# HandSomeWay/myGauHuman

Hardware: AMD Instinct MI355X
Metric: frames/sec fwd+bwd @1024^2, 200k Gaussians (higher is better)
Workload: dtype f32

## Files before the change

include/gsr.h:

```cpp
#ifndef GSR_H_INCLUDED
#define GSR_H_INCLUDED

#include <stddef.h>
#include <stdint.h>

#ifdef __cplusplus
extern "C" {
#endif

#define GSR_OK 0
#define GSR_EINVAL (-1)
#define GSR_EHIP (-2)
#define GSR_ENOMEM (-3)

typedef void *gsr_stream_t;
typedef char *(*gsr_alloc_fn)(void *user, size_t bytes);

int gsr_version(void);
int gsr_has_experiments(void);
const char *gsr_target_arch(void);
const char *gsr_last_error(void);

#define GSR_BINNING_GLOBAL_RADIX 0
#define GSR_BINNING_TILE_BUCKET 1
// ... 117 lines not shown

#define GSR_Q_DEPTHS 0
#define GSR_Q_MEANS2D 1
#define GSR_Q_CONIC_OPACITY 2
#define GSR_Q_RGB 3
#define GSR_Q_COV3D 4
#define GSR_Q_TILES_TOUCHED 5
#define GSR_Q_POINT_OFFSETS 6
#define GSR_Q_CLAMPED 7
#define GSR_Q_POINT_LIST 8
#define GSR_Q_KEYS_SORTED 9
#define GSR_Q_RANGES 10
#define GSR_Q_FINAL_T 11
#define GSR_Q_N_CONTRIB 12
#define GSR_Q_ORDER 13
int gsr_query_state(int what, int P, int R, int width, int height, const char *geom_buffer,
                    const char *binning_buffer, const char *image_buffer, void *dst, gsr_stream_t stream);

size_t gsr_dist2_workspace_bytes(int P);
int gsr_dist2(int P, const float *points, float *mean_dists, char *workspace, size_t workspace_bytes,
              gsr_stream_t stream);

size_t gsr_sort_workspace_bytes(size_t n);
int gsr_sort_pairs_u64(size_t n, const uint64_t *keys_in, uint64_t *keys_out, const uint32_t *vals_in,
                       uint32_t *vals_out, int end_bit, char *workspace, size_t workspace_bytes,
                       gsr_stream_t stream);
int gsr_sort_pairs_u32(size_t n, const uint32_t *keys_in, uint32_t *keys_out, const uint32_t *vals_in,
                       uint32_t *vals_out, int end_bit, char *workspace, size_t workspace_bytes,
                       gsr_stream_t stream);

// ... 291 lines not shown
```

mygauhuman_amd/_lib.py:

```python
import ctypes as C
import os

import torch

_HERE = os.path.dirname(os.path.abspath(__file__))
LIB_PATH = os.path.join(_HERE, "libgsr.so")

ALLOC_FN = C.CFUNCTYPE(C.c_void_p, C.c_void_p, C.c_size_t)


class Phase1LossStruct(C.Structure):
    _fields_ = [("gt_image", C.c_void_p), ("gt_normal", C.c_void_p), ("alpha_target", C.c_void_p), ("bound", C.c_void_p),
                ("w_image", C.c_float), ("w_alpha", C.c_float), ("w_normal", C.c_float), ("w_axis", C.c_float),
                ("normal_triple", C.c_int), ("axis_triple", C.c_int),
                ("color", C.c_void_p), ("alpha", C.c_void_p), ("extra_images", C.c_void_p), ("stats", C.c_void_p),
                ("upstream", C.c_void_p)]

PBR_MAX_LEVELS = 16


class PbrTexture(C.Structure):
    _fields_ = [("cube", C.c_int), ("channels", C.c_int), ("levels", C.c_int),
                ("width", C.c_int * PBR_MAX_LEVELS), ("height", C.c_int * PBR_MAX_LEVELS),
                ("data", C.c_void_p * PBR_MAX_LEVELS), ("grad", C.c_void_p * PBR_MAX_LEVELS)]
# ... 47 lines not shown
    "gsr_body_pose_backward", "gsr_lbs_offset_mlp_packed_floats_nb", "gsr_lbs_offset_mlp_pack_nb", "gsr_lbs_offset_mlp_forward_nb",
    "gsr_debug_lbs_offset_mlp_forward_bf16x3_nb", "gsr_lbs_offset_mlp_backward_workspace_floats_nb", "gsr_lbs_offset_mlp_backward_nb",
    "gsr_pbr_texture_forward", "gsr_pbr_texture_backward", "gsr_pbr_cube_mip_forward", "gsr_pbr_cube_mip_backward",
    "gsr_pbr_diffuse_forward", "gsr_pbr_diffuse_backward", "gsr_pbr_specular_forward", "gsr_pbr_specular_backward",
    "gsr_pbr_shade_forward", "gsr_pbr_shade_backward",
    "gsr_bake_grid_workspace_bytes", "gsr_bake_grid", "gsr_bake_plan_bytes", "gsr_bake_plan", "gsr_bake_visibility_workspace_bytes",
    "gsr_bake_visibility", "gsr_bake_expand", "gsr_bake_env_reduce",
    "gsr_pbr_loss_workspace_floats", "gsr_pbr_loss_forward", "gsr_pbr_loss_backward",
    "gsr_pose_refiner_forward", "gsr_pose_refiner_backward",
    "gsr_bounding_rect_workspace_ints", "gsr_bounding_rect", "gsr_ssim_crop_workspace_floats", "gsr_ssim_crop_forward",
    "gsr_ssim_crop_backward",
]

GSR_OK = 0
Q = dict(DEPTHS=0, MEANS2D=1, CONIC_OPACITY=2, RGB=3, COV3D=4, TILES_TOUCHED=5, POINT_OFFSETS=6, CLAMPED=7,
         POINT_LIST=8, KEYS_SORTED=9, RANGES=10, FINAL_T=11, N_CONTRIB=12, ORDER=13)
BINNING_GLOBAL_RADIX, BINNING_TILE_BUCKET = 0, 1
SH_F32, SH_F16 = 0, 1
N_EXTRA = 18
DEFAULT_BINNING = BINNING_TILE_BUCKET
DEFAULT_TILE_CULL = 1
DEFAULT_BWD_REDUCE = 3
DEFAULT_TILE_ORDER = 1
DEFAULT_BLEND_LAYOUT = 0
DEFAULT_BLEND_SEGMENTS = 8


class GsrError(RuntimeError):
    pass


# ... 250 lines not shown
```

mygauhuman_amd/csrc/blend_bwd.hip:

```cpp
#include "gsr_common.h"

namespace gsr {

__device__ __forceinline__ uint32_t xcd_remap_b(uint32_t bid, uint32_t n) {
  const uint32_t q = n / 8, r = n % 8, xcd = bid % 8, k = bid / 8;
  const uint32_t start = xcd < r ? xcd * (q + 1) : r * (q + 1) + (xcd - r) * q;
  return start + k;
}

template <int CTRL>
__device__ __forceinline__ float dpp_f(float v) {
  return __builtin_bit_cast(float, __builtin_amdgcn_update_dpp(0, __builtin_bit_cast(int, v), CTRL, 0xF, 0xF, false));
}
__device__ __forceinline__ float row16_sum(float v) {
  v += dpp_f<0xB1>(v);
  v += dpp_f<0x4E>(v);
  v += dpp_f<0x124>(v);
  v += dpp_f<0x128>(v);
  return v;
}
__device__ __forceinline__ float half8_sum(float v) {
  v += dpp_f<0xB1>(v);
  v += dpp_f<0x4E>(v);
  v += dpp_f<0x141>(v);
// ... 575 lines not shown
    dps[ch][1] = t4.y;
    dps[ch][2] = t4.z;
    dps[ch][3] = t4.w;
  }
  __builtin_amdgcn_wave_barrier();
  const float4 *rd_r = reinterpret_cast<const float4 *>(&s_rw[row * WAVE + kcol * 4u]);
  const float4 *rd_w = reinterpret_cast<const float4 *>(&s_rw[(4u + row) * WAVE + kcol * 4u]);
  constexpr uint32_t H2_QA = 68, H2_QB = 0, H2_QC = 132, H2_KA = 224, H2_KB = 292;
  constexpr uint64_t H2_P = ((uint64_t)(H2_QB / 4)) | ((uint64_t)((H2_QA + 8) / 4) << 7) | ((uint64_t)(H2_QC / 4) << 14) |
                            ((uint64_t)((H2_QB + 8) / 4) << 21) | ((uint64_t)((H2_QC + 8) / 4) << 28) | ((uint64_t)(H2_QA / 4) << 35) |
                            ((uint64_t)(H2_KA / 4) << 42) | ((uint64_t)((H2_KA + 8) / 4) << 49) | ((uint64_t)(H2_KB / 4) << 56);
  static_assert((H2_KB + WAVE) * 4 <= RW_BYTES, "hop 2 fits the reduction buffer");
  const uint32_t k9 = kcol < 9u ? kcol : 0u;
  const float4 *src8 = reinterpret_cast<const float4 *>(&s_rw[row * 16u + 4u * (uint32_t)((H2_P >> (7u * k9)) & 127u)]);

  uint32_t id_next = 0;
  if (skip + (int)lane < walk_end) id_next = a.point_list[range.y - 1 - (skip + (int)lane)];
  for (int base = skip; base < walk_end; base += WAVE) {
    const int idx = base + (int)lane;
    bool keep = false;
    float4 r0 = make_float4(0, 0, 0, 0), r1 = r0, r2 = r0;
    float l255 = 0.f;
    const uint32_t id = id_next;
    if (idx < walk_end) {
      const float4 *src = reinterpret_cast<const float4 *>(a.recs + id);
      r0 = src[0];
      r1 = src[1];
      r2 = src[2];
    }
    if (idx + WAVE < walk_end) id_next = a.point_list[range.y - 1 - (idx + WAVE)];
    if (idx < walk_end) {
      keep = (r0.x + r2.z >= rx0) && (r0.x - r2.z <= rx1) && (r0.y + r2.w >= ry0) && (r0.y - r2.w <= ry1);
      if (keep) {
        l255 = __builtin_amdgcn_logf(255.0f * r1.y);
        keep = ellipse_hits_rect_fast(r0.x, r0.y, r0.z, r0.w, r1.x, l255, rx0, rx1, ry0, ry1);
      }
    }
    const uint64_t kmask = __ballot(keep);
    const int cnt = __builtin_popcountll(kmask);
    if (keep) {
      const int slot = __builtin_popcountll(kmask & lt);
      constexpr float L2E = 1.4426950408889634f;
      s0[slot] = make_float4(r0.x, r0.y, (-0.5f * L2E) * r0.z, -L2E * r0.w);
      s1[slot] = make_float4((-0.5f * L2E) * r1.x, l255, __uint_as_float((uint32_t)(n - 1 - idx)), r1.y);
      s2[slot] = make_float4(r1.w, r2.x, r2.y, r1.z);
      s_id[slot] = id * (uint32_t)(GROW * sizeof(float));
    }
    __builtin_amdgcn_fence(__ATOMIC_RELEASE, "wavefront");
    __builtin_amdgcn_wave_barrier();
    __builtin_amdgcn_fence(__ATOMIC_ACQUIRE, "wavefront");

    uint32_t vg = 0u, vi = row * 4u;
    asm volatile("" : "+v"(vg), "+v"(vi));
    for (int g = 0; g < cnt; g += 4, vg += 64u, vi += 16u) {
      float ar[4], aw[4];
      uint32_t anyhit = 0;
#pragma unroll
      for (int u = 0; u < 4; u++) {
        bool done = false;
        if (g + u < cnt) {
          const float4 g0 = lds_at<float4>(s0, vg + 16u * u);
// ... 768 lines not shown
```

mygauhuman_amd/csrc/blend_fwd.hip:

```cpp
#include "gsr_common.h"
#include "tile_sort.h"

#ifndef FWD_FULL_ROWS
#define FWD_FULL_ROWS false
#endif
#ifndef FWD_FEATURE_WPG
#define FWD_FEATURE_WPG 2
#endif

namespace gsr {

__device__ __forceinline__ uint32_t xcd_remap(uint32_t bid, uint32_t n) {
  const uint32_t q = n / 8, r = n % 8, xcd = bid % 8, k = bid / 8;
  const uint32_t start = xcd < r ? xcd * (q + 1) : r * (q + 1) + (xcd - r) * q;
  return start + k;
}

template <int SLOTS, int CE>
constexpr int fwd_wpg() { return SLOTS == 1 ? (CE > 0 ? FWD_FEATURE_WPG : 4) : 1; }

__device__ __forceinline__ void workgroup_sort_tile(const uint64_t *b, int n, uint32_t tile, uint32_t base, uint32_t *point_list,
                                                    uint64_t *keys_sorted, uint32_t wv, uint32_t lane, uint64_t *s_runs,
                                                    uint32_t *s_ids) {
  const int nruns = (n + WAVE - 1) / WAVE, r0 = (int)wv, r1 = (int)wv + 4;
// ... 19 lines not shown
    if (r >= nruns) break;
    const uint64_t k = key[j];
    uint32_t rank = lane;
#pragma unroll
    for (int o = 0; o < MERGE_MAX_RUNS; o++)
      if (o != r && o < nruns) rank += rank_in_run(s_runs + o * WAVE, k);
    if (k != ~0ull) {
      point_list[base + rank] = (uint32_t)k;
      keys_sorted[base + rank] = ((uint64_t)tile << 32) | (k >> 32);
      s_ids[rank] = (uint32_t)k;
    }
  }
  __syncthreads();
}

template <int SLOTS, int CE>
__global__ __launch_bounds__((WAVE * fwd_wpg<SLOTS, CE>())) void blend_forward_kernel(const BlendFwdArgs a) {
  constexpr int WPG = fwd_wpg<SLOTS, CE>();
  constexpr uint32_t H = SLOTS == 1 ? 4 / WPG : 1;
  const uint32_t wv = threadIdx.x / WAVE;
  constexpr int WPT = 4 / SLOTS;
  constexpr int XS2 = CE > 0 ? (CE + 3) / 4 * 2 : 1;
  __shared__ __attribute__((aligned(16))) float2 s_x_all[CE > 0 ? WPG * WAVE * XS2 : 1];
  __shared__ float4 s0_all[WPG * WAVE];
  __shared__ float4 s1_all[WPG * WAVE];
  __shared__ float4 s2_all[WPG * WAVE];
  float2 *s_x = s_x_all + (CE > 0 ? wv * WAVE * XS2 : 0);
  float4 *s0 = s0_all + wv * WAVE, *s1 = s1_all + wv * WAVE, *s2 = s2_all + wv * WAVE;

  const unsigned long long trace_t0 = a.trace ? __builtin_amdgcn_s_memrealtime() : 0ull;
  uint32_t tile, part, nseg = 1;
  if constexpr (SLOTS == 1) {
// ... 46 lines not shown
    const int q = q0 + s;
    const int px = tx * TILE + (q & 1) * 8 + (int)(lane & 7);
    const int py = ty * TILE + (q >> 1) * 8 + (int)(lane >> 3);
    pxf[s] = (float)px;
    pyf[s] = (float)py;
    inside[s] = px < a.W && py < a.H;
    dbias[s] = inside[s] ? -0.02f : 1e30f;
    pixid[s] = py * a.W + px;
    T[s] = 1.0f;
    C0[s] = C1[s] = C2[s] = Dp[s] = Wt[s] = 0.f;
#pragma unroll
    for (int c = 0; c < (CE > 0 ? CE : 1); c++) X[s][c] = 0.f;
    last[s] = 0;
  }
  const uint64_t lt = lane == 0 ? 0ull : (~0ull >> (64 - lane));

  uint32_t id_a = 0, id_b = 0;
  float4 p0 = make_float4(0, 0, 0, 0), p1 = p0, p2 = p0;
  uint32_t id_cur = 0;
  if ((int)lane < n) {
    id_cur = list_at((int)lane);
    const float4 *src = reinterpret_cast<const float4 *>(a.recs + id_cur);
    p0 = src[0];
    p1 = src[1];
    p2 = src[2];
  }
  if ((int)lane + WAVE < n) id_a = list_at((int)lane + WAVE);
  const int seg_len = nseg > 1u ? segment_len(n, (int)nseg) : 0;
  uint32_t next_rec = 0;
  auto checkpoint = [&](uint32_t k) {
// ... 65 lines not shown
    };
    auto fetch_rest = [&](Row &r) {
      r.g2 = s2[r.kk];
      if (CE > 0) {
        const float4 *xr = reinterpret_cast<const float4 *>(&s_x[r.kk * XS2]);
#pragma unroll
        for (int c = 0; c < XS2 / 2; c++) r.x[c] = xr[c];
      }
    };
    auto fetch = [&](Row &r, int k) {
      r.kk = min(k, WAVE - 1);
      r.g0 = s0[r.kk];
      r.g1 = s1[r.kk];
      if constexpr (FULL) fetch_rest(r);
    };
    auto blend_one = [&](Row &r) {
#pragma unroll
      for (int s = 0; s < SLOTS; s++) {
        const float dx = r.g0.x - pxf[s], dy = r.g0.y - pyf[s];
        const float p2 = dx * (r.g0.z * dx + r.g0.w * dy) + (r.g1.x * dy) * dy;
        const bool pre = !(p2 > 0.0f) && ((p2 + r.g1.y) >= dbias[s]);
        if (__ballot(pre) != 0ull) {
          if constexpr (!FULL) fetch_rest(r);
          const float alpha = fminf(0.99f, r.g1.w * __builtin_amdgcn_exp2f(p2));
          const bool hit = pre && !(alpha < 1.0f / 255.0f);
          const float test_T = T[s] * (1.0f - alpha);
          const bool stop = hit && test_T < 0.0001f;
          const bool blend = hit && !stop;
          dbias[s] = stop ? 1e30f : dbias[s];
          const float w = blend ? alpha * T[s] : 0.0f;
          C0[s] += r.g2.x * w;
          C1[s] += r.g2.y * w;
          C2[s] += r.g2.z * w;
          Dp[s] += r.g2.w * w;
          Wt[s] += w;
          if (CE > 0) {
#pragma unroll
            for (int c = 0; c < CE; c++) {
              const float4 v = r.x[c / 4];
              X[s][c] += (c % 4 == 0 ? v.x : (c % 4 == 1 ? v.y : (c % 4 == 2 ? v.z : v.w))) * w;
            }
          }
          T[s] = blend ? test_T : T[s];
          last[s] = blend ? __float_as_uint(r.g1.z) : last[s];
        }
      }
    };
    Row A, B;
    fetch(A, 0);
    int k = 0;
    for (; k + 1 < cnt; k += 2) {
      fetch(B, k + 1);
      blend_one(A);
      fetch(A, k + 2);
      blend_one(B);
    }
    if (k < cnt) blend_one(A);
    __builtin_amdgcn_wave_barrier();
  }
  if (nseg > 1u)
    while (next_rec < nseg) checkpoint(next_rec++);
  if (a.trace && lane == 0) {
    unsigned long long *r = a.trace + ((size_t)blockIdx.x * WPG + wv) * 4u;
    r[0] = trace_t0;
    r[1] = __builtin_amdgcn_s_memrealtime();
    r[2] = (unsigned long long)n;
    r[3] = (unsigned long long)tile;
  }

  const size_t plane = (size_t)a.H * a.W;
  const float bg0 = a.bg[0], bg1 = a.bg[1], bg2 = a.bg[2];
#pragma unroll
// ... 27 lines not shown

constexpr int FX_PLANE16 = WAVE * 16;
constexpr int FX_BYTES = 4 * FX_PLANE16 + 2 * WAVE * 4;
constexpr int HALF = WAVE / 2;

__global__ __launch_bounds__(WAVE * 4) void blend_forward_features_kernel(const BlendFwdArgs a) {
  constexpr int CE = CE_MAX;
  const uint32_t wv = threadIdx.x / WAVE;
  __shared__ __attribute__((aligned(16))) char s_fx_all[4 * FX_BYTES];
  __shared__ float4 s0_all[4 * WAVE], s1_all[4 * WAVE], s2_all[4 * WAVE];
  __shared__ uint32_t s_lane_all[4 * WAVE];
  char *s_fx = s_fx_all + wv * FX_BYTES;
  float4 *s0w = s0_all + wv * WAVE, *s1w = s1_all + wv * WAVE, *s2w = s2_all + wv * WAVE;
  uint32_t *s_lanew = s_lane_all + wv * WAVE;
  const uint32_t fx_base = __builtin_amdgcn_readfirstlane((uint32_t)(uintptr_t)s_fx);

  const int omode = tile_order_mode(a.order);
  const uint32_t n_slots = tile_slots_of(a.order, a.grid_x, a.grid_y, omode);
  const uint32_t slot_id = omode ? blockIdx.x : (blockIdx.x < n_slots ? xcd_remap(blockIdx.x, n_slots) : n_slots);
  const uint32_t entry = tile_of_slot(a.order, omode, slot_id, n_slots), part = wv;
  if (entry == ORDER_NO_TILE || order_entry_seg(entry) != 0u) return;
  const uint32_t tile = order_entry_tile(entry);
  const int tx = tile % a.grid_x, ty = tile / a.grid_x;
  const uint32_t lane = threadIdx.x % WAVE;
  const uint2 range = a.ranges[tile];
  const int n = (int)(range.y - range.x);
  list_priority(a.order, n, a.list_prio);

  const int px = tx * TILE + (int)(part & 1) * 8 + (int)(lane & 7);
  const int py = ty * TILE + (int)(part >> 1) * 8 + (int)(lane >> 3);
// ... 142 lines not shown
  const uint32_t s = max(h.x, h.y);
  const fwd_u32x2 q = __builtin_amdgcn_permlane16_swap(s, s, false, false);
  return max(q.x, q.y);
}

template <int CE>
__global__ __launch_bounds__(WAVE * 4) void blend_forward_sp_kernel(const BlendFwdArgs a) {
  constexpr int XS = (CE + 3) / 4 * 4;
  __shared__ float4 s_x_all[CE > 0 ? 4 * WAVE * XS / 4 : 1];
  __shared__ float4 s0_all[4 * WAVE];
  __shared__ float4 s1_all[4 * WAVE];
  __shared__ float4 s2_all[4 * WAVE];
  const uint32_t wv = threadIdx.x / WAVE, lane = threadIdx.x % WAVE;
  float4 *s_x = s_x_all + (CE > 0 ? wv * WAVE * XS / 4 : 0);
  float4 *s0 = s0_all + wv * WAVE, *s1 = s1_all + wv * WAVE, *s2 = s2_all + wv * WAVE;

  const int omode = tile_order_mode(a.order);
  const uint32_t n_slots = tile_slots_of(a.order, a.grid_x, a.grid_y, omode);
  const uint32_t item = omode ? ordered_item4(blockIdx.x, n_slots) : (blockIdx.x < n_slots * 4u ? xcd_remap(blockIdx.x, n_slots * 4u) : n_slots * 4u);
  const uint32_t entry = tile_of_slot(a.order, omode, item / 4u, n_slots), quad = item % 4u;
  if (entry == ORDER_NO_TILE || order_entry_seg(entry) != 0u) return;
  const uint32_t tile = order_entry_tile(entry);
  const int tx = tile % a.grid_x, ty = tile / a.grid_x;
  const uint2 range = a.ranges[tile];
  const int n = (int)(range.y - range.x);
  list_priority(a.order, n, a.list_prio);

  s2[lane] = make_float4(0.f, 0.f, 0.f, 0.f);
  if (CE > 0) {
#pragma unroll
// ... 186 lines not shown
      return GSR_OK;
    }
#endif
    hipLaunchKernelGGL((blend_forward_kernel<1, CE_MAX>), dim3(slots * (4 / FWD_FEATURE_WPG)), dim3(WAVE * FWD_FEATURE_WPG), 0, stream, a);
    return GSR_OK;
  }
#ifdef GSR_BUILD_EXPERIMENTS
  if (opt.blend_layout == 1 && opt.blend_fwd_waves == 4) {
    hipLaunchKernelGGL((blend_forward_sp_kernel<0>), dim3(slots * 4), dim3(WAVE * 4), 0, stream, a);
    return GSR_OK;
  }
#endif
  switch (opt.blend_fwd_waves) {
    case 1: hipLaunchKernelGGL((blend_forward_kernel<4, 0>), dim3(tiles), dim3(WAVE), 0, stream, a); break;
    case 2: hipLaunchKernelGGL((blend_forward_kernel<2, 0>), dim3(tiles * 2), dim3(WAVE), 0, stream, a); break;
    default: hipLaunchKernelGGL((blend_forward_kernel<1, 0>), dim3(slots), dim3(WAVE * 4), 0, stream, a); break;
  }
  return GSR_OK;
}

}
```

mygauhuman_amd/csrc/gsr_api.hip:

```cpp
#include <stdarg.h>
#include <stdio.h>
#include <string.h>

#include <atomic>
#include <mutex>
#include <string>
#include <unordered_map>
#include <utility>
#include <vector>

#include "gsr_common.h"

namespace gsr {

static thread_local std::string g_error;

void set_error(const char *fmt, ...) {
  char buf[1024];
  va_list ap;
  va_start(ap, fmt);
  vsnprintf(buf, sizeof(buf), fmt, ap);
  va_end(ap);
  g_error = buf;
}
// ... 79 lines not shown
  } else if (!strcmp(key, "blend_bwd_waves")) {
    if (v != 1 && v != 2 && v != 4) return bad("1, 2 or 4");
    o.blend_bwd_waves = v;
  } else if (!strcmp(key, "bucket_cstride")) {
    if (v != 1 && v != 2 && v != 4 && v != 8 && v != 16) return bad("1, 2, 4, 8 or 16");
    o.bucket_cstride = v;
  } else if (!strcmp(key, "bucket_hist")) {
    if (v != 0 && v != 1) return bad("0 or 1");
    o.bucket_hist = v;
  } else if (!strcmp(key, "bucket_sort_merged")) {
    if (v != 0 && v != 1) return bad("0 or 1");
    o.bucket_sort_merged = v;
  } else if (!strcmp(key, "blend_sort")) {
    if (v != 0 && v != 1) return bad("0 or 1");
    o.blend_sort = v;
  } else if (!strcmp(key, "tile_order")) {
    if (v < 0 || v > 3) return bad("0 (natural order), 1 (longest lists first), 2 / 3 (2 x 2 / 4 x 2 tile blocks by summed length, a block per XCD)");
    o.tile_order = v;
  } else if (!strcmp(key, "tile_cull")) {
    if (v != 0 && v != 1) return bad("0 or 1");
    o.tile_cull = v;
  } else if (!strcmp(key, "blend_bwd_reduce")) {
    if (v < 0 || v > 4) return bad("0 (permlane / DPP folds), 3 (LDS folds: default); experiments: 1 (MFMA on folded rows), 2 (transposed MFMA contraction), 4 (LDS folds, the round-3 kernel)");
    if (experiment(v == 1 || v == 2 || v == 4)) return GSR_EINVAL;
    o.blend_bwd_reduce = v;
  } else if (!strcmp(key, "blend_layout")) {
    if (v != 0 && v != 1) return bad("0 (quadrant waves) or 1 (experiment: 4x4 blocks, four survivors per step)");
    if (experiment(v == 1)) return GSR_EINVAL;
    o.blend_layout = v;
  } else if (!strcmp(key, "blend_tail_cut")) {
// ... 336 lines not shown
  fa.W = in.width;
  fa.H = in.height;
  fa.grid_x = grid_x;
  fa.grid_y = grid_y;
  fa.bg = in.background;
  fa.out_color = in.out_color;
  fa.out_depth = in.out_depth;
  fa.out_alpha = in.out_alpha;
  fa.final_T = img.final_T;
  fa.n_contrib = img.n_contrib;
  fa.extra = in.extra;
  fa.CE = in.n_extra;
  fa.list_prio = opt.blend_prio;
  fa.ckpt_base = img.ckpt_base;
  fa.ckpt = img.ckpt;
  {
    ApiState &st = S();
    const size_t need = (size_t)tile_slots_max(grid_x, grid_y) * 4u * 4u;
    fa.trace = st.trace.load();
    if (fa.trace && st.trace_words.load() / 2 < need) {
      set_error("gsr_debug_wave_trace: the registered buffer holds %zu words, this image needs %zu (2 x 16 x visiting slots)",
                st.trace_words.load(), 2 * need);
      return GSR_EINVAL;
    }
  }
  fa.out_extra = in.out_extra;
  prof_begin(PROF_BLEND_FWD, stream);
  rc = launch_blend_forward(fa, opt, stream);
  prof_end(PROF_BLEND_FWD, stream);
  if (rc != GSR_OK) return rc;
// ... 166 lines not shown
  }
  if (p1 && (n_extra != CE_MAX || !p1->gt_image || !p1->gt_normal || !p1->alpha_target || !p1->bound || !p1->color || !p1->alpha ||
             !p1->extra_images || !p1->stats || p1->normal_triple < 0 || p1->normal_triple > 5 || p1->axis_triple < 0 ||
             p1->axis_triple > 5 || p1->axis_triple == p1->normal_triple)) {
    set_error("gsr_rasterize_backward_phase1_loss: the fused multi-feature pass (n_extra = %d), the forward's images, the targets, "
              "the bound mask, stats and two different triple indices in 0..5 are required", CE_MAX);
    return GSR_EINVAL;
  }
  if ((shs && !dL_dsh) || (scales && (!rotations || !dL_dscale || !dL_drot))) {
    set_error("gsr_rasterize_backward: missing gradient output for SH / scale / rotation inputs");
    return GSR_EINVAL;
  }
  const int grid_x = (width + TILE - 1) / TILE, grid_y = (height + TILE - 1) / TILE;
  const size_t tiles = (size_t)grid_x * grid_y, npix = (size_t)width * height;
  GeomState geom = geom_from_chunk(geom_buffer, (size_t)P);
  BinningState bin = binning_from_chunk(binning_buffer, (size_t)R);
  ImageState img = image_from_chunk(image_buffer, npix, tiles);
  if (!radii) radii = geom.internal_radii;

  if (n_extra != 0 && (n_extra != CE_MAX || !extra_features || !dL_dout_extra || !dL_dextra)) {
    set_error("gsr_rasterize_backward_ex: extra feature channels need n_extra == %d and all three arrays", CE_MAX);
    return GSR_EINVAL;
  }
  const int grow = n_extra ? GROWX : GROW;
  const Options opt = options_for(stream);
  float *det_rows = nullptr;
  const size_t det_bytes = (size_t)(R > 0 ? R : 1) * 4 * GROW * sizeof(float);
  if (opt.deterministic) {
    GSR_HIP(hipMalloc(reinterpret_cast<void **>(&det_rows), det_bytes));
    GSR_HIP(zero_async(det_rows, det_bytes, stream));
  } else if (!(flags & GSR_BWD_ROWS_ZEROED)) {
// ... 29 lines not shown
    if (ba.dL_dextra_tri[t]) ba.extra_mask |= 1u << t;
  }
  if (p1) {
    ba.p1 = *p1;
    ba.extra_mask |= (1u << p1->normal_triple) | (1u << p1->axis_triple);
    if (opt.deterministic || opt.blend_bwd_reduce != 3) {
      set_error("gsr_rasterize_backward_phase1_loss: built for the default reduction of the fused pass (blend_bwd_reduce = 3, not deterministic)");
      return GSR_EINVAL;
    }
  }
  ba.det_rows = det_rows;
  ba.debug_skip_atomics = opt.debug_no_atomics;
  ba.list_prio = opt.blend_prio;
  ba.ckpt_base = img.ckpt_base;
  ba.ckpt = img.ckpt;
  {
    ApiState &st = S();
    const size_t need = (size_t)tile_slots_max(ba.grid_x, ba.grid_y) * 4u * 4u;
    ba.trace = st.trace.load() ? st.trace.load() + st.trace_words.load() / 2 : nullptr;
    if (ba.trace && st.trace_words.load() / 2 < need) {
      set_error("gsr_debug_wave_trace: the registered buffer holds %zu words, this image needs %zu (2 x 16 x visiting slots)",
                st.trace_words.load(), 2 * need);
      return GSR_EINVAL;
    }
  }
  ba.radii = radii;
  ba.point_offsets = geom.point_offsets;
  ba.tiles_touched = geom.tiles_touched;
  prof_begin(PROF_BLEND_BWD, stream);
  int rc = launch_blend_backward(ba, opt, stream);
// ... 126 lines not shown
                           float *dL_dscale, float *dL_drot, int debug, gsr_stream_t stream) {
  return gsr_rasterize_backward_ex(P, D, M, R, background, width, height, means3D, shs, colors_precomp, alphas, scales,
                                   scale_modifier, rotations, cov3D_precomp, viewmatrix, projmatrix, campos, tan_fovx, tan_fovy,
                                   radii, geom_buffer, binning_buffer, image_buffer, dL_dpix, dL_ddepths, dL_dalphas, dL_dmean2D,
                                   dL_dconic, dL_dopacity, dL_dcolor, dL_dmean3D, dL_dcov3D, dL_dsh, dL_dscale, dL_drot, debug,
                                   nullptr, 0, nullptr, nullptr, GSR_SH_F32, stream);
}

int gsr_query_state(int what, int P, int R, int width, int height, const char *geom_buffer, const char *binning_buffer,
                    const char *image_buffer, void *dst, gsr_stream_t stream_) {
  hipStream_t stream = reinterpret_cast<hipStream_t>(stream_);
  const int grid_x = (width + TILE - 1) / TILE, grid_y = (height + TILE - 1) / TILE;
  const size_t tiles = (size_t)grid_x * grid_y, npix = (size_t)width * height;
  if (!dst) return GSR_EINVAL;
  GeomState geom = geom_from_chunk(const_cast<char *>(geom_buffer), (size_t)P);
  BinningState bin = binning_from_chunk(const_cast<char *>(binning_buffer), (size_t)R);
  ImageState img = image_from_chunk(const_cast<char *>(image_buffer), npix, tiles);
  const void *src = nullptr;
  size_t bytes = 0;
  switch (what) {
    case GSR_Q_DEPTHS:
    case GSR_Q_MEANS2D:
    case GSR_Q_CONIC_OPACITY:
    case GSR_Q_RGB:
    case GSR_Q_CLAMPED: {
      if (!geom_buffer) return GSR_EINVAL;
      int rc = launch_query_recs(what, P, geom, dst, stream);
      if (rc != GSR_OK) return rc;
      GSR_LAUNCH_CHECK(stream, 0);
      return GSR_OK;
    }
    case GSR_Q_COV3D: src = geom.cov3D; bytes = (size_t)P * 6 * 4; break;
    case GSR_Q_TILES_TOUCHED: src = geom.tiles_touched; bytes = (size_t)P * 4; break;
    case GSR_Q_POINT_OFFSETS: src = geom.point_offsets; bytes = (size_t)P * 4; break;
    case GSR_Q_POINT_LIST: src = bin.vals_s; bytes = (size_t)R * 4; break;
    case GSR_Q_KEYS_SORTED: src = bin.keys_s; bytes = (size_t)R * 8; break;
    case GSR_Q_RANGES: src = img.ranges; bytes = tiles * 8; break;
    case GSR_Q_FINAL_T: src = img.final_T; bytes = npix * 4; break;
    case GSR_Q_N_CONTRIB: src = img.n_contrib; bytes = npix * 4; break;
    case GSR_Q_ORDER: src = img.order; bytes = order_words(tiles) * 4; break;
    default: set_error("gsr_query_state: unknown selector %d", what); return GSR_EINVAL;
  }
  if (bytes) GSR_HIP(hipMemcpyAsync(dst, src, bytes, hipMemcpyDeviceToDevice, stream));
  return GSR_OK;
}

size_t gsr_sort_workspace_bytes(size_t n) {
  size_t m = n ? n : 1;
  return align_up(m * 8, 256) + align_up(m * 4, 256) + align_up(sort_hist_words(m) * 4, 256) + 1024;
}

static int sort_ws(size_t n, size_t key_bytes, char *ws, size_t ws_bytes, void **tk, uint32_t **tv, uint32_t **hist) {
  if (!ws || ws_bytes < gsr_sort_workspace_bytes(n)) {
    set_error("sort workspace too small (%zu < %zu)", ws_bytes, gsr_sort_workspace_bytes(n));
    return GSR_ENOMEM;
// ... 48 lines not shown
```

mygauhuman_amd/csrc/gsr_common.h:

```cpp
#pragma once
#include <hip/hip_runtime.h>
#include <stdint.h>
#include <stddef.h>

#include "../../include/gsr.h"

namespace gsr {

constexpr int TILE = 16;
constexpr int WAVE = 64;
constexpr int PRE_BLOCK = 256;

struct alignas(16) SplatRec {
  float x, y, conic_a, conic_b;
  float conic_c, opacity, depth, r;
  float g, b, hx, hy;
};
static_assert(sizeof(SplatRec) == 48, "SplatRec layout");

constexpr int GROW = 16;

constexpr int GROWX = 32;
constexpr int CE_MAX = 18;

// ... 6 lines not shown
  int *internal_radii;
  uint32_t *block_incl;
  uint32_t *block_sums;
  uint32_t *block_prefix;
  uint32_t *total;
  float *grad_rows;
};
struct BinningState {
  uint64_t *keys_a;
  uint32_t *vals_a;
  uint64_t *keys_s;
  uint32_t *vals_s;
  uint32_t *hist;
  uint32_t *tile_counts;
  uint32_t *tile_cursor;
};
struct ImageState {
  float *final_T;
  uint32_t *n_contrib;
  uint2 *ranges;
  uint32_t *order;
  uint32_t *ckpt_base;
  float *ckpt;
};

inline size_t align_up(size_t v, size_t a) { return (v + a - 1) / a * a; }
template <typename T>
inline void carve(uintptr_t &p, T *&out, size_t count) {
  p = align_up(p, 256);
  out = reinterpret_cast<T *>(p);
// ... 19 lines not shown
  carve(chunk, g.point_offsets, P);
  carve(chunk, g.internal_radii, P);
  carve(chunk, g.block_incl, P);
  carve(chunk, g.block_sums, nb);
  carve(chunk, g.block_prefix, nb);
  carve(chunk, g.total, 4);
  carve(chunk, g.grad_rows, P * GROWX);
  if (end) *end = chunk;
  return g;
}
inline size_t geom_bytes(size_t P) {
  size_t end = 0;
  geom_from_chunk(nullptr, P, &end);
  return end + 256;
}
inline BinningState binning_from_chunk(char *chunk_, size_t R, size_t tiles = 0, size_t *end = nullptr) {
  BinningState b;
  uintptr_t chunk = carve_begin(chunk_);
  size_t n = R ? R : 1;
  carve(chunk, b.keys_a, n);
  carve(chunk, b.vals_a, n);
  carve(chunk, b.keys_s, n);
  carve(chunk, b.vals_s, n);
  carve(chunk, b.hist, sort_hist_words(n));
  b.tile_counts = b.tile_cursor = nullptr;
  if (tiles) {
    carve(chunk, b.tile_counts, tiles * 16);
    carve(chunk, b.tile_cursor, tiles);
  }
  if (end) *end = chunk;
  return b;
}
inline size_t binning_bytes(size_t R, size_t tiles) {
  size_t end = 0;
  binning_from_chunk(nullptr, R, tiles ? tiles : 1, &end);
  return end + 256;
}
#if defined(__HIPCC__)
#define GSR_HD __host__ __device__
#else
#define GSR_HD
#endif
constexpr uint32_t ORDER_NO_TILE = 0xFFFFFFFFu;
// ... 56 lines not shown
    if (debug) GSR_HIP(hipStreamSynchronize(stream));                        \
  } while (0)

enum ProfStage { PROF_PREPROCESS_FWD = 0, PROF_SCAN = 1, PROF_BINNING = 2, PROF_BLEND_FWD = 3, PROF_BLEND_BWD = 4,
                 PROF_PREPROCESS_BWD = 5, PROF_NSTAGES = 6 };
void prof_begin(int stage, hipStream_t stream);
void prof_end(int stage, hipStream_t stream);

struct Options {
  int binning_mode = GSR_BINNING_TILE_BUCKET;
  int tile_cull = 1;
  int tile_order = 1;
  int bucket_hist = 1;
  int bucket_sort_merged = 1;
  int blend_sort = 1;
  int bucket_cstride = 4;
  int blend_fwd_dma = 0;
  int blend_fwd_waves = 4;
  int blend_bwd_waves = 4;
  int blend_bwd_reduce = 3;
  int deterministic = 0;
  int blend_layout = 0;
  int blend_tail_cut = 0;
  int blend_segments = 8;
  int blend_prio = 1;
  int bake_batch_cells = 0;
  int debug_no_atomics = 0;
};
Options options_for(hipStream_t stream);

// ... 27 lines not shown
  const uint2 *ranges;
  uint32_t *point_list;
  const SplatRec *recs;
  const uint64_t *unsorted;
  uint64_t *keys_sorted;
  int W, H, grid_x, grid_y;
  const float *bg;
  float *out_color, *out_depth, *out_alpha, *final_T;
  uint32_t *n_contrib;
  const float *extra;
  int CE;
  float *out_extra;
  int list_prio;
  const uint32_t *ckpt_base;
  float *ckpt;
  unsigned long long *trace;
};
int launch_blend_forward(const BlendFwdArgs &a, const Options &opt, hipStream_t stream);
bool forward_sorts_lists(const Options &opt, int n_extra);
__device__ __forceinline__ int tile_order_mode(const uint32_t *order) { return order ? (int)(order[0] & 0xFFu) : 0; }
__device__ __forceinline__ uint32_t tile_order_longest(const uint32_t *order) { return order ? order[0] >> 8 : 0u; }
__device__ __forceinline__ void list_priority(const uint32_t *order, int n, int enabled) {
  const uint32_t longest = tile_order_longest(order), n4 = 4u * (uint32_t)n;
  if (!enabled || longest == 0u) return;
#ifdef GSR_BUILD_EXPERIMENTS
  if (enabled >= 2 && n4 < (uint32_t)(enabled == 2 ? 3 : (enabled == 3 ? 2 : 1)) * longest) __builtin_amdgcn_endpgm();
#endif
  if (n4 >= 3u * longest) __builtin_amdgcn_s_setprio(3);
  else if (n4 >= 2u * longest) __builtin_amdgcn_s_setprio(2);
  else if (n4 >= longest) __builtin_amdgcn_s_setprio(1);
// ... 23 lines not shown
  const uint32_t *n_contrib;
  const float *dL_dpix, *dL_ddepth, *dL_dalpha;
  const float *loss_color, *loss_alpha, *loss_gt, *loss_mask;
  float loss_sc, loss_sa;
  float *grad_rows;
  const float *extra;
  int CE;
  const float *dL_dextra_tri[CE_MAX / 3];
  uint32_t extra_mask;
  float *det_rows;
  const int *radii;
  const uint32_t *point_offsets, *tiles_touched;
  int list_prio;
  const uint32_t *ckpt_base;
  const float *ckpt;
  unsigned long long *trace;
  int debug_skip_atomics;
  gsr_phase1_loss p1;
};
int launch_reduce_det_rows(int P, const uint32_t *point_offsets, const uint32_t *tiles_touched, const float *det_rows,
                           size_t n_slots, float *grad_rows, hipStream_t stream);
int launch_blend_backward(const BlendBwdArgs &a, const Options &opt, hipStream_t stream);

struct PreprocessBwdArgs {
  int P, D, M;
  const float *means3D, *shs, *scales, *rotations, *cov3D;
  const int *radii;
  const uint8_t *clamped;
  float scale_modifier;
  const float *view, *proj, *campos;
// ... 117 lines not shown
```

mygauhuman_amd/diff_gaussian_rasterization/_C.py:

```python
import contextlib
import ctypes as C

import torch

from .. import _lib
from .._lib import ALLOC_FN, check, lib, ptr
from ..fastpath import DeferredStatus


def _f32c(t, name):
    if t.numel() and t.dtype != torch.float32:
        raise RuntimeError(f"{name} must be float32")
    return t.contiguous()


def _sh(t):
    if t.numel() and t.dtype == torch.float16:
        return t.contiguous(), _lib.SH_F16
    return _f32c(t, "sh"), _lib.SH_F32


def _stream(device):
    return torch.cuda.current_stream(device).cuda_stream

# ... 312 lines not shown
    if P != 0:
        means3D, viewmatrix, projmatrix = _f32c(means3D, "means3D"), _f32c(viewmatrix, "viewmatrix"), _f32c(projmatrix, "projmatrix")
        with torch.cuda.device(means3D.device):
            check(lib.gsr_mark_visible(P, ptr(means3D), ptr(viewmatrix), ptr(projmatrix), present.data_ptr(),
                                       _stream(means3D.device)), "gsr_mark_visible")
    return present


def query_state(what, P, R, W, H, geomBuffer, binningBuffer, imageBuffer):
    dev = geomBuffer.device
    tiles = ((W + 15) // 16) * ((H + 15) // 16)
    shapes = dict(DEPTHS=((P,), torch.float32), MEANS2D=((P, 2), torch.float32), CONIC_OPACITY=((P, 4), torch.float32),
                  RGB=((P, 3), torch.float32), COV3D=((P, 6), torch.float32), TILES_TOUCHED=((P,), torch.int32),
                  POINT_OFFSETS=((P,), torch.int32), CLAMPED=((P, 3), torch.uint8), POINT_LIST=((R,), torch.int32),
                  KEYS_SORTED=((R,), torch.int64), RANGES=((tiles, 2), torch.int32), FINAL_T=((H, W), torch.float32),
                  N_CONTRIB=((H, W), torch.int32), ORDER=((4 * tiles + 66,), torch.int32))
    shape, dt = shapes[what]
    out = torch.zeros(shape, dtype=dt, device=dev)
    if out.numel():
        with torch.cuda.device(dev):
            check(lib.gsr_query_state(_lib.Q[what], P, R, W, H, geomBuffer.data_ptr(),
                                      binningBuffer.data_ptr() if binningBuffer.numel() else None,
                                      imageBuffer.data_ptr(), out.data_ptr(), _stream(dev)), "gsr_query_state")
    return out
```

Before: 2887.

## Record per-wave blend contribution bitmasks in forward to skip culling in backward

The plain four-wave forward blend kernel now writes, for each 64-entry chunk of a tile's list and each wave part, a bitmask of the Gaussians that actually blended for some pixel. A stamp word marks the masks as valid. The backward walk reads these masks instead of re-running the bounding-box and ellipse cull. It packs only the contributing entries into shared memory, walking chunks from the top down. This removes redundant culling work and record loads in backward, at the cost of extra binning buffer space, mask writes and ballots in forward, and a new default-on option.

```diff
diff --git a/include/gsr.h b/include/gsr.h
--- a/include/gsr.h
+++ b/include/gsr.h
@@ -155,6 +155,7 @@
 #define GSR_Q_FINAL_T 11
 #define GSR_Q_N_CONTRIB 12
 #define GSR_Q_ORDER 13
+#define GSR_Q_BLEND_BITS 14
 int gsr_query_state(int what, int P, int R, int width, int height, const char *geom_buffer,
                     const char *binning_buffer, const char *image_buffer, void *dst, gsr_stream_t stream);
 
diff --git a/mygauhuman_amd/_lib.py b/mygauhuman_amd/_lib.py
--- a/mygauhuman_amd/_lib.py
+++ b/mygauhuman_amd/_lib.py
@@ -85,7 +85,7 @@
 
 GSR_OK = 0
 Q = dict(DEPTHS=0, MEANS2D=1, CONIC_OPACITY=2, RGB=3, COV3D=4, TILES_TOUCHED=5, POINT_OFFSETS=6, CLAMPED=7,
-         POINT_LIST=8, KEYS_SORTED=9, RANGES=10, FINAL_T=11, N_CONTRIB=12, ORDER=13)
+         POINT_LIST=8, KEYS_SORTED=9, RANGES=10, FINAL_T=11, N_CONTRIB=12, ORDER=13, BLEND_BITS=14)
 BINNING_GLOBAL_RADIX, BINNING_TILE_BUCKET = 0, 1
 SH_F32, SH_F16 = 0, 1
 N_EXTRA = 18
diff --git a/mygauhuman_amd/csrc/blend_bwd.hip b/mygauhuman_amd/csrc/blend_bwd.hip
--- a/mygauhuman_amd/csrc/blend_bwd.hip
+++ b/mygauhuman_amd/csrc/blend_bwd.hip
@@ -613,37 +613,82 @@
   const uint32_t k9 = kcol < 9u ? kcol : 0u;
   const float4 *src8 = reinterpret_cast<const float4 *>(&s_rw[row * 16u + 4u * (uint32_t)((H2_P >> (7u * k9)) & 127u)]);
 
+  const int hi = n - skip;
+  const bool use_bits = a.bits && hi > s_lo && a.bits[0] == BITS_STAMP;
+  const uint64_t *brow = a.bits + BITS_HDR + 4u * (size_t)(range.x / 64u + tile) + part;
+  const int c_hi = use_bits ? (hi - 1) >> 6 : 0;
+  const int nit = use_bits ? c_hi - (s_lo >> 6) + 1 : (walk_end - skip + WAVE - 1) / WAVE;
   uint32_t id_next = 0;
-  if (skip + (int)lane < walk_end) id_next = a.point_list[range.y - 1 - (skip + (int)lane)];
-  for (int base = skip; base < walk_end; base += WAVE) {
-    const int idx = base + (int)lane;
-    bool keep = false;
-    float4 r0 = make_float4(0, 0, 0, 0), r1 = r0, r2 = r0;
-    float l255 = 0.f;
-    const uint32_t id = id_next;
-    if (idx < walk_end) {
-      const float4 *src = reinterpret_cast<const float4 *>(a.recs + id);
-      r0 = src[0];
-      r1 = src[1];
-      r2 = src[2];
-    }
-    if (idx + WAVE < walk_end) id_next = a.point_list[range.y - 1 - (idx + WAVE)];
-    if (idx < walk_end) {
-      keep = (r0.x + r2.z >= rx0) && (r0.x - r2.z <= rx1) && (r0.y + r2.w >= ry0) && (r0.y - r2.w <= ry1);
+  uint64_t m_cur = 0ull, m_next = 0ull;
+  if (use_bits) {
+    const int top = hi - (c_hi << 6);
+    m_cur = brow[4 * c_hi] & (top >= 64 ? ~0ull : ((1ull << top) - 1ull));
+    if (nit > 1) m_next = brow[4 * (c_hi - 1)];
+    if ((m_cur >> lane) & 1ull) id_next = a.point_list[range.x + (uint32_t)(c_hi << 6) + lane];
+  } else if (skip + (int)lane < walk_end) {
+    id_next = a.point_list[range.y - 1 - (skip + (int)lane)];
+  }
+  for (int it = 0; it < nit;) {
+    int cnt;
+    constexpr float L2E = 1.4426950408889634f;
+    if (use_bits) {
+      cnt = 0;
+      do {
+      const int c = c_hi - it;
+      const uint64_t m = m_cur;
+      const bool mine = ((m >> lane) & 1ull) != 0ull;
+      const int pc = __builtin_popcountll(m);
+      const uint32_t id = id_next;
+      float4 r0 = make_float4(0, 0, 0, 0), r1 = r0, r2 = r0;
+      if (mine) {
+        const float4 *src = reinterpret_cast<const float4 *>(a.recs + id);
+        r0 = src[0];
+        r1 = src[1];
+        r2 = src[2];
+      }
+      m_cur = m_next;
+      m_next = it + 2 < nit ? brow[4 * (c - 2)] : 0ull;
+      if ((m_cur >> lane) & 1ull) id_next = a.point_list[range.x + (uint32_t)((c - 1) << 6) + lane];
+      if (mine) {
+        const int slot = cnt + pc - 1 - __builtin_popcountll(m & lt);
+        s0[slot] = make_float4(r0.x, r0.y, (-0.5f * L2E) * r0.z, -L2E * r0.w);
+        s1[slot] = make_float4((-0.5f * L2E) * r1.x, __builtin_amdgcn_logf(255.0f * r1.y), __uint_as_float((uint32_t)((c << 6) + (int)lane)), r1.y);
+        s2[slot] = make_float4(r1.w, r2.x, r2.y, r1.z);
+        s_id[slot] = id * (uint32_t)(GROW * sizeof(float));
+      }
+      cnt += pc;
+      it++;
+      } while (it < nit && cnt + __builtin_popcountll(m_cur) <= WAVE);
+    } else {
+      const int idx = skip + it * WAVE + (int)lane;
+      bool keep = false;
+      float4 r0 = make_float4(0, 0, 0, 0), r1 = r0, r2 = r0;
+      float l255 = 0.f;
+      const uint32_t id = id_next;
+      if (idx < walk_end) {
+        const float4 *src = reinterpret_cast<const float4 *>(a.recs + id);
+        r0 = src[0];
+        r1 = src[1];
+        r2 = src[2];
+      }
+      if (idx + WAVE < walk_end) id_next = a.point_list[range.y - 1 - (idx + WAVE)];
+      if (idx < walk_end) {
+        keep = (r0.x + r2.z >= rx0) && (r0.x - r2.z <= rx1) && (r0.y + r2.w >= ry0) && (r0.y - r2.w <= ry1);
+        if (keep) {
+          l255 = __builtin_amdgcn_logf(255.0f * r1.y);
+          keep = ellipse_hits_rect_fast(r0.x, r0.y, r0.z, r0.w, r1.x, l255, rx0, rx1, ry0, ry1);
+        }
+      }
+      const uint64_t kmask = __ballot(keep);
+      cnt = __builtin_popcountll(kmask);
       if (keep) {
-        l255 = __builtin_amdgcn_logf(255.0f * r1.y);
-        keep = ellipse_hits_rect_fast(r0.x, r0.y, r0.z, r0.w, r1.x, l255, rx0, rx1, ry0, ry1);
-      }
-    }
-    const uint64_t kmask = __ballot(keep);
-    const int cnt = __builtin_popcountll(kmask);
-    if (keep) {
-      const int slot = __builtin_popcountll(kmask & lt);
-      constexpr float L2E = 1.4426950408889634f;
-      s0[slot] = make_float4(r0.x, r0.y, (-0.5f * L2E) * r0.z, -L2E * r0.w);
-      s1[slot] = make_float4((-0.5f * L2E) * r1.x, l255, __uint_as_float((uint32_t)(n - 1 - idx)), r1.y);
-      s2[slot] = make_float4(r1.w, r2.x, r2.y, r1.z);
-      s_id[slot] = id * (uint32_t)(GROW * sizeof(float));
+        const int slot = __builtin_popcountll(kmask & lt);
+        s0[slot] = make_float4(r0.x, r0.y, (-0.5f * L2E) * r0.z, -L2E * r0.w);
+        s1[slot] = make_float4((-0.5f * L2E) * r1.x, l255, __uint_as_float((uint32_t)(n - 1 - idx)), r1.y);
+        s2[slot] = make_float4(r1.w, r2.x, r2.y, r1.z);
+        s_id[slot] = id * (uint32_t)(GROW * sizeof(float));
+      }
+      it++;
     }
     __builtin_amdgcn_fence(__ATOMIC_RELEASE, "wavefront");
     __builtin_amdgcn_wave_barrier();
diff --git a/mygauhuman_amd/csrc/blend_fwd.hip b/mygauhuman_amd/csrc/blend_fwd.hip
--- a/mygauhuman_amd/csrc/blend_fwd.hip
+++ b/mygauhuman_amd/csrc/blend_fwd.hip
@@ -57,8 +57,10 @@
   __syncthreads();
 }
 
-template <int SLOTS, int CE>
+template <int SLOTS, int CE, bool BITS = false>
 __global__ __launch_bounds__((WAVE * fwd_wpg<SLOTS, CE>())) void blend_forward_kernel(const BlendFwdArgs a) {
+  static_assert(!BITS || (SLOTS == 1 && CE == 0), "blend masks: plain four-wave forward only");
+  if (a.bits && blockIdx.x == 0 && threadIdx.x == 0) a.bits[0] = BITS ? BITS_STAMP : 0ull;
   constexpr int WPG = fwd_wpg<SLOTS, CE>();
   constexpr uint32_t H = SLOTS == 1 ? 4 / WPG : 1;
   const uint32_t wv = threadIdx.x / WAVE;
@@ -135,6 +137,7 @@
     last[s] = 0;
   }
   const uint64_t lt = lane == 0 ? 0ull : (~0ull >> (64 - lane));
+  const uint32_t bits_w0 = BITS ? __builtin_amdgcn_readfirstlane((uint32_t)BITS_HDR + 4u * (range.x / 64u + tile) + part) : 0u;
 
   uint32_t id_a = 0, id_b = 0;
   float4 p0 = make_float4(0, 0, 0, 0), p1 = p0, p2 = p0;
@@ -230,7 +233,8 @@
       r.g1 = s1[r.kk];
       if constexpr (FULL) fetch_rest(r);
     };
-    auto blend_one = [&](Row &r) {
+    uint64_t cbits = 0ull;
+    auto blend_one = [&](Row &r, int k) {
 #pragma unroll
       for (int s = 0; s < SLOTS; s++) {
         const float dx = r.g0.x - pxf[s], dy = r.g0.y - pyf[s];
@@ -259,6 +263,8 @@
           }
           T[s] = blend ? test_T : T[s];
           last[s] = blend ? __float_as_uint(r.g1.z) : last[s];
+          if constexpr (BITS)
+            cbits |= __builtin_amdgcn_ballot_w64(blend) != 0ull ? 1ull << k : 0ull;
         }
       }
     };
@@ -267,11 +273,16 @@
     int k = 0;
     for (; k + 1 < cnt; k += 2) {
       fetch(B, k + 1);
-      blend_one(A);
+      blend_one(A, k);
       fetch(A, k + 2);
-      blend_one(B);
-    }
-    if (k < cnt) blend_one(A);
+      blend_one(B, k + 1);
+    }
+    if (k < cnt) blend_one(A, k);
+    if constexpr (BITS) {
+      const bool mine = keep && ((cbits >> __builtin_popcountll(kmask & lt)) & 1ull) != 0ull;
+      const uint64_t word = __ballot(mine);
+      if (lane == 0) a.bits[bits_w0 + 4u * (uint32_t)(base / WAVE)] = word;
+    }
     __builtin_amdgcn_wave_barrier();
   }
   if (nseg > 1u)
@@ -329,6 +340,7 @@
   float4 *s0w = s0_all + wv * WAVE, *s1w = s1_all + wv * WAVE, *s2w = s2_all + wv * WAVE;
   uint32_t *s_lanew = s_lane_all + wv * WAVE;
   const uint32_t fx_base = __builtin_amdgcn_readfirstlane((uint32_t)(uintptr_t)s_fx);
+  if (a.bits && blockIdx.x == 0 && threadIdx.x == 0) a.bits[0] = 0ull;
 
   const int omode = tile_order_mode(a.order);
   const uint32_t n_slots = tile_slots_of(a.order, a.grid_x, a.grid_y, omode);
@@ -501,6 +513,7 @@
   const uint32_t wv = threadIdx.x / WAVE, lane = threadIdx.x % WAVE;
   float4 *s_x = s_x_all + (CE > 0 ? wv * WAVE * XS / 4 : 0);
   float4 *s0 = s0_all + wv * WAVE, *s1 = s1_all + wv * WAVE, *s2 = s2_all + wv * WAVE;
+  if (a.bits && blockIdx.x == 0 && threadIdx.x == 0) a.bits[0] = 0ull;
 
   const int omode = tile_order_mode(a.order);
   const uint32_t n_slots = tile_slots_of(a.order, a.grid_x, a.grid_y, omode);
@@ -717,7 +730,10 @@
   switch (opt.blend_fwd_waves) {
     case 1: hipLaunchKernelGGL((blend_forward_kernel<4, 0>), dim3(tiles), dim3(WAVE), 0, stream, a); break;
     case 2: hipLaunchKernelGGL((blend_forward_kernel<2, 0>), dim3(tiles * 2), dim3(WAVE), 0, stream, a); break;
-    default: hipLaunchKernelGGL((blend_forward_kernel<1, 0>), dim3(slots), dim3(WAVE * 4), 0, stream, a); break;
+    default:
+      if (opt.blend_bits && a.bits) hipLaunchKernelGGL((blend_forward_kernel<1, 0, true>), dim3(slots), dim3(WAVE * 4), 0, stream, a);
+      else hipLaunchKernelGGL((blend_forward_kernel<1, 0>), dim3(slots), dim3(WAVE * 4), 0, stream, a);
+      break;
   }
   return GSR_OK;
 }
diff --git a/mygauhuman_amd/csrc/gsr_api.hip b/mygauhuman_amd/csrc/gsr_api.hip
--- a/mygauhuman_amd/csrc/gsr_api.hip
+++ b/mygauhuman_amd/csrc/gsr_api.hip
@@ -117,6 +117,9 @@
   } else if (!strcmp(key, "blend_sort")) {
     if (v != 0 && v != 1) return bad("0 or 1");
     o.blend_sort = v;
+  } else if (!strcmp(key, "blend_bits")) {
+    if (v != 0 && v != 1) return bad("0 or 1");
+    o.blend_bits = v;
   } else if (!strcmp(key, "tile_order")) {
     if (v < 0 || v > 3) return bad("0 (natural order), 1 (longest lists first), 2 / 3 (2 x 2 / 4 x 2 tile blocks by summed length, a block per XCD)");
     o.tile_order = v;
@@ -483,6 +486,7 @@
   fa.list_prio = opt.blend_prio;
   fa.ckpt_base = img.ckpt_base;
   fa.ckpt = img.ckpt;
+  fa.bits = bin.blend_bits;
   {
     ApiState &st = S();
     const size_t need = (size_t)tile_slots_max(grid_x, grid_y) * 4u * 4u;
@@ -679,7 +683,7 @@
   const int grid_x = (width + TILE - 1) / TILE, grid_y = (height + TILE - 1) / TILE;
   const size_t tiles = (size_t)grid_x * grid_y, npix = (size_t)width * height;
   GeomState geom = geom_from_chunk(geom_buffer, (size_t)P);
-  BinningState bin = binning_from_chunk(binning_buffer, (size_t)R);
+  BinningState bin = binning_from_chunk(binning_buffer, (size_t)R, tiles);
   ImageState img = image_from_chunk(image_buffer, npix, tiles);
   if (!radii) radii = geom.internal_radii;
 
@@ -739,6 +743,7 @@
   ba.list_prio = opt.blend_prio;
   ba.ckpt_base = img.ckpt_base;
   ba.ckpt = img.ckpt;
+  ba.bits = opt.blend_bits ? bin.blend_bits : nullptr;
   {
     ApiState &st = S();
     const size_t need = (size_t)tile_slots_max(ba.grid_x, ba.grid_y) * 4u * 4u;
@@ -895,7 +900,7 @@
   const size_t tiles = (size_t)grid_x * grid_y, npix = (size_t)width * height;
   if (!dst) return GSR_EINVAL;
   GeomState geom = geom_from_chunk(const_cast<char *>(geom_buffer), (size_t)P);
-  BinningState bin = binning_from_chunk(const_cast<char *>(binning_buffer), (size_t)R);
+  BinningState bin = binning_from_chunk(const_cast<char *>(binning_buffer), (size_t)R, tiles);
   ImageState img = image_from_chunk(const_cast<char *>(image_buffer), npix, tiles);
   const void *src = nullptr;
   size_t bytes = 0;
@@ -920,6 +925,7 @@
     case GSR_Q_FINAL_T: src = img.final_T; bytes = npix * 4; break;
     case GSR_Q_N_CONTRIB: src = img.n_contrib; bytes = npix * 4; break;
     case GSR_Q_ORDER: src = img.order; bytes = order_words(tiles) * 4; break;
+    case GSR_Q_BLEND_BITS: src = bin.blend_bits; bytes = blend_bits_words((size_t)(R > 0 ? R : 1), tiles) * 8; break;
     default: set_error("gsr_query_state: unknown selector %d", what); return GSR_EINVAL;
   }
   if (bytes) GSR_HIP(hipMemcpyAsync(dst, src, bytes, hipMemcpyDeviceToDevice, stream));
diff --git a/mygauhuman_amd/csrc/gsr_common.h b/mygauhuman_amd/csrc/gsr_common.h
--- a/mygauhuman_amd/csrc/gsr_common.h
+++ b/mygauhuman_amd/csrc/gsr_common.h
@@ -44,6 +44,7 @@
   uint32_t *hist;
   uint32_t *tile_counts;
   uint32_t *tile_cursor;
+  uint64_t *blend_bits;
 };
 struct ImageState {
   float *final_T;
@@ -93,6 +94,10 @@
   geom_from_chunk(nullptr, P, &end);
   return end + 256;
 }
+constexpr uint64_t BITS_STAMP = 0x626c656e64626974ull;
+constexpr size_t BITS_HDR = 4;
+inline size_t blend_bits_words(size_t R, size_t tiles) { return BITS_HDR + 4 * (R / 64 + tiles + 2); }
+
 inline BinningState binning_from_chunk(char *chunk_, size_t R, size_t tiles = 0, size_t *end = nullptr) {
   BinningState b;
   uintptr_t chunk = carve_begin(chunk_);
@@ -103,9 +108,11 @@
   carve(chunk, b.vals_s, n);
   carve(chunk, b.hist, sort_hist_words(n));
   b.tile_counts = b.tile_cursor = nullptr;
+  b.blend_bits = nullptr;
   if (tiles) {
     carve(chunk, b.tile_counts, tiles * 16);
     carve(chunk, b.tile_cursor, tiles);
+    carve(chunk, b.blend_bits, blend_bits_words(n, tiles));
   }
   if (end) *end = chunk;
   return b;
@@ -192,6 +199,7 @@
   int bucket_hist = 1;
   int bucket_sort_merged = 1;
   int blend_sort = 1;
+  int blend_bits = 1;
   int bucket_cstride = 4;
   int blend_fwd_dma = 0;
   int blend_fwd_waves = 4;
@@ -249,6 +257,7 @@
   int list_prio;
   const uint32_t *ckpt_base;
   float *ckpt;
+  uint64_t *bits;
   unsigned long long *trace;
 };
 int launch_blend_forward(const BlendFwdArgs &a, const Options &opt, hipStream_t stream);
@@ -302,6 +311,7 @@
   int list_prio;
   const uint32_t *ckpt_base;
   const float *ckpt;
+  const uint64_t *bits;
   unsigned long long *trace;
   int debug_skip_atomics;
   gsr_phase1_loss p1;
diff --git a/mygauhuman_amd/diff_gaussian_rasterization/_C.py b/mygauhuman_amd/diff_gaussian_rasterization/_C.py
--- a/mygauhuman_amd/diff_gaussian_rasterization/_C.py
+++ b/mygauhuman_amd/diff_gaussian_rasterization/_C.py
@@ -350,7 +350,8 @@
                   RGB=((P, 3), torch.float32), COV3D=((P, 6), torch.float32), TILES_TOUCHED=((P,), torch.int32),
                   POINT_OFFSETS=((P,), torch.int32), CLAMPED=((P, 3), torch.uint8), POINT_LIST=((R,), torch.int32),
                   KEYS_SORTED=((R,), torch.int64), RANGES=((tiles, 2), torch.int32), FINAL_T=((H, W), torch.float32),
-                  N_CONTRIB=((H, W), torch.int32), ORDER=((4 * tiles + 66,), torch.int32))
+                  N_CONTRIB=((H, W), torch.int32), ORDER=((4 * tiles + 66,), torch.int32),
+                  BLEND_BITS=((4 + 4 * (max(R, 1) // 64 + tiles + 2),), torch.int64))
     shape, dt = shapes[what]
     out = torch.zeros(shape, dtype=dt, device=dev)
     if out.numel():
```

New measurement: 2731. 0.946x the previous value.
